# labRadioVision/federated

Hardware: AMD Instinct MI355X
Metric: device-resident GB/s, CFA reduce of K neighbour fp32 param buckets; 1/2/4/8 GPU (higher is better)
Workload: dtype f32

## Files before the change

### federated_amd/csrc/cfa_internal.h

```cpp
#pragma once
#include <hip/hip_runtime.h>

#include <cmath>
#include <cstdarg>
#include <cstdint>
#include <cstdio>
#include <cstdlib>
#include <cstring>
#include <string>
#include <type_traits>
#include <utility>

#include "cfa_engine.h"
#include "cfa_mix_shape.h"

typedef float f4 __attribute__((ext_vector_type(4)));
typedef unsigned u4v __attribute__((ext_vector_type(4)));

inline thread_local std::string g_last_error;

__attribute__((format(printf, 2, 3))) inline int fail(int code, const char* fmt, ...) {
  char buf[512];
  va_list ap;
  va_start(ap, fmt);
  vsnprintf(buf, sizeof(buf), fmt, ap);
  va_end(ap);
  g_last_error = buf;
  return code;
}

#define CFA_HIP_CHECK(expr)                                                              \
  do {                                                                                   \
    hipError_t e_ = (expr);                                                              \
    if (e_ != hipSuccess)                                                                \
      return fail(CFA_E_HIP, "%s failed: %s (%s:%d)", #expr, hipGetErrorString(e_),      \
                  __FILE__, __LINE__);                                                   \
  } while (0)

inline int check_launch(const char* what) {
  hipError_t e = hipGetLastError();
  if (e != hipSuccess) return fail(CFA_E_HIP, "%s launch failed: %s", what, hipGetErrorString(e));
  return CFA_OK;
}

namespace {

constexpr int kBlock = 256;

constexpr int kDefaultBlocks = 2;
constexpr int kAutoBlocks = -1;
static cfa_launch_t read_tune() {
  cfa_launch_t t{kAutoBlocks, 0, 1};
  if (const char* s = getenv("CFA_BLOCKS_PER_CU")) {
    const int v = atoi(s);
    t.blocks_per_cu = v >= 0 ? v : kAutoBlocks;
  }
  if (const char* s = getenv("CFA_VEC_PER_LANE")) t.vec_per_lane = norm_vec(atoi(s));
  if (const char* s = getenv("CFA_NONTEMPORAL")) t.nontemporal = atoi(s) ? 1 : 0;
  return t;
}
static const cfa_launch_t& tune() {
  static const cfa_launch_t t = read_tune();
  static const bool dynamic = getenv("CFA_TUNE_DYNAMIC") != nullptr;
  if (dynamic) {
    thread_local cfa_launch_t d;
    d = read_tune();
    return d;
  }
  return t;
}

}

inline int device_attr(int slot, hipDeviceAttribute_t attr, int fallback, bool keep_fallback) {
  static int cache[2][64] = {{0}};
  int dev = 0;
  if (hipGetDevice(&dev) != hipSuccess) return fallback;
  if (dev >= 0 && dev < 64) {
    const int c = __atomic_load_n(&cache[slot][dev], __ATOMIC_RELAXED);
    if (c > 0) return c;
  }
  int v = 0;
  if (hipDeviceGetAttribute(&v, attr, dev) != hipSuccess || v <= 0) {
    if (!keep_fallback) return fallback;
    v = fallback;
  }
  if (dev >= 0 && dev < 64) __atomic_store_n(&cache[slot][dev], v, __ATOMIC_RELAXED);
  return v;
}
inline int device_cus() { return device_attr(0, hipDeviceAttributeMultiprocessorCount, 256, false); }
inline int device_lds_max() { return device_attr(1, hipDeviceAttributeMaxSharedMemoryPerBlock, 65536, true); }

int grad_prepare_device();
int local_sgd_prepare_device();
int lenet_prepare_device();
int lenet_grad_prepare_device();
int advance_counter(unsigned long long* counter, hipStream_t st);

namespace {

static unsigned grid_for(long long tiles, const cfa_launch_t& t = tune()) {
  if (tiles <= 0) return 1;
  long long g = tiles;
  const int bpc = t.blocks_per_cu == kAutoBlocks ? kDefaultBlocks : t.blocks_per_cu;
  if (bpc > 0) {
    long long cap = (long long)device_cus() * bpc;
    if (g > cap) g = cap;
  }
  if (g > 0x7fffffffLL) g = 0x7fffffffLL;
  return (unsigned)g;
}

static unsigned grid_for_own(long long tiles, int own_blocks_per_cu) {
  cfa_launch_t t = tune();
  if (t.blocks_per_cu == kAutoBlocks) t.blocks_per_cu = own_blocks_per_cu;
  return grid_for(tiles, t);
}

static unsigned shared_grid_x(long long tiles, int wg_per_cu, long long gy) {
  long long gx = ((long long)device_cus() * wg_per_cu + gy - 1) / gy;
  if (gx > tiles) gx = tiles;
  if (gx < 1) gx = 1;
  return (unsigned)gx;
}

static int env_int(const char* name, int unset) {
  const char* s = getenv(name);
  return s ? atoi(s) : unset;
}

struct Fanin {
  const float* src[CFA_MAX_FANIN + 1];
  float c[CFA_MAX_FANIN + 1];
  float d[CFA_MAX_FANIN + 1];
  double rd[CFA_MAX_FANIN + 1];
};

constexpr int kFcSubnormal = 0x0090;
__device__ __forceinline__ f4 div4_rn(f4 a, double rb, bool& subnormal) {
  f4 q;
  q.x = (float)((double)a.x * rb);
  q.y = (float)((double)a.y * rb);
  q.z = (float)((double)a.z * rb);
  q.w = (float)((double)a.w * rb);
  subnormal = subnormal | __builtin_isfpclass(q.x, kFcSubnormal) | __builtin_isfpclass(q.y, kFcSubnormal) |
              __builtin_isfpclass(q.z, kFcSubnormal) | __builtin_isfpclass(q.w, kFcSubnormal);
  return q;
}
__device__ __forceinline__ f4 div4_ieee(f4 a, float b) {
  f4 q;
  q.x = a.x / b;
  q.y = a.y / b;
  q.z = a.z / b;
  q.w = a.w / b;
  return q;
}

inline void set_reciprocals(Fanin& f, int n) {
  for (int k = 0; k <= n; ++k) f.rd[k] = 1.0 / (double)f.d[k];
}

template <bool NT>
__device__ __forceinline__ f4 ld4(const float* p, long long i) {
  const f4* q = reinterpret_cast<const f4*>(p) + i;
  if constexpr (NT) return __builtin_nontemporal_load(q);
  else return *q;
}
template <bool NT>
__device__ __forceinline__ void st4(float* p, long long i, f4 v) {
  f4* q = reinterpret_cast<f4*>(p) + i;
  if constexpr (NT) __builtin_nontemporal_store(v, q);
  else *q = v;
}

template <typename T>
__device__ __forceinline__ T seq_step(T acc, T x, float a) {
  T t = x - acc;
  t = a * t;
  return acc + t;
}

template <bool IEEE, typename T>
__device__ __forceinline__ T div_step(T w, T x, float c, float d, double rd, bool& subnormal) {
  T t = x - w;
  t = c * t;
  if constexpr (!IEEE) t = div4_rn(t, rd, subnormal);
  else if constexpr (std::is_same_v<T, f4>) t = div4_ieee(t, d);
  else t = t / d;
  return w + t;
}

template <typename T>
__device__ __forceinline__ T lin_step(T w, T x, float c) {
  if constexpr (std::is_same_v<T, float>) {
    return fmaf(c, x, w);
  } else {
    w.x = fmaf(c, x.x, w.x);
    w.y = fmaf(c, x.y, w.y);
    w.z = fmaf(c, x.z, w.z);
    w.w = fmaf(c, x.w, w.w);
    return w;
  }
}

template <typename L>
__device__ __forceinline__ double tf1_first(L l, float x, double a) {
  const float d = x - (float)l;
  return (double)l + a * (double)d;
}
template <typename X>
__device__ __forceinline__ double tf1_step(double w, X x, double a) {
  return w + a * ((double)x - w);
}

__device__ __forceinline__ double ddiv_rn(double a, double b, double rb, bool fast) {
  const double aa = __builtin_fabs(a);
  if (fast && aa >= 0x1p-900 && aa <= 0x1p900) {
    const double q = a * rb;
    const double r = __builtin_fma(-q, b, a);
    return __builtin_fma(r, rb, q);
  }
  return a / b;
}
template <bool IEEE>
__device__ __forceinline__ double div_step_f64(double w, double x, double a, double d, double r, bool fast) {
  if constexpr (IEEE) return w + (a * (x - w)) / d;
  else return w + ddiv_rn(a * (x - w), d, r, fast);
}

template <typename T>
__device__ __forceinline__ T mewma_step(T& W, T g, const T& s_old, float rho, float one_minus_rho, T lr, bool init,
                                        bool filtered) {
  T s;
  if (init) {
    s = g;
  } else {
    const T t1 = rho * g;
    const T t2 = one_minus_rho * s_old;
    s = t1 + t2;
  }
  const T u = lr * (filtered ? s : g);
  W = W - u;
  return s;
}

__device__ __forceinline__ double scale(double c, double x, bool f32) {
  return f32 ? (double)((float)c * (float)x) : c * x;
}
__device__ __forceinline__ double mewma_step_f64(double& W, bool& w32, double g, const double& s_old, double rho,
                                                 double one_minus_rho, double lr, bool init, bool filtered,
                                                 bool s32, bool g32) {
  double s;
  if (init) {
    s = g;
  } else {
    const double t1 = scale(rho, g, g32);
    const double t2 = scale(one_minus_rho, s_old, s32);
    s = (g32 && s32) ? (double)((float)t1 + (float)t2) : t1 + t2;
  }
  if (s32) s = (double)(float)s;
  const bool u32 = filtered ? s32 : g32;
  const double t = scale(lr, filtered ? s : g, u32);
  if (w32 && u32) {
    W = (double)((float)W - (float)t);
  } else {
    W = W - t;
    w32 = false;
  }
  return s;
}

__device__ __forceinline__ float split_sum(const float* p, int n, long long stride) {
  float s = p[0];
  for (int sp = 1; sp < n; ++sp) s += p[(long long)sp * stride];
  return s;
}

template <int N, bool IEEE>
__device__ __forceinline__ f4 fold_div(const f4 (&v)[N + 1], const Fanin& f, bool& subnormal) {
  f4 w = v[0];
#pragma unroll
  for (int j = 1; j <= N; ++j) w = div_step<IEEE>(w, v[j], f.c[j], f.d[j], f.rd[j], subnormal);
  return w;
}

template <int N, int RULE>
__device__ __forceinline__ f4 fold(const f4 (&v)[N + 1], const Fanin& f) {
  if constexpr (RULE == CFA_RULE_SEQUENTIAL) {
    f4 w = v[0];
#pragma unroll
    for (int j = 1; j <= N; ++j) w = seq_step(w, v[j], f.c[j]);
    return w;
  } else if constexpr (RULE == CFA_RULE_SEQUENTIAL_DIV) {
    bool subnormal = false;
    f4 w = fold_div<N, false>(v, f, subnormal);
    if (__builtin_expect(subnormal, 0)) w = fold_div<N, true>(v, f, subnormal);
    return w;
  } else {
    f4 w = f.c[0] * v[0];
#pragma unroll
    for (int j = 1; j <= N; ++j) w = lin_step(w, v[j], f.c[j]);
    return w;
  }
}

template <int U>
struct TileWalk {
  static constexpr long long kTile = (long long)kBlock * U;
  long long nvec, full;
  __device__ explicit TileWalk(long long n) : nvec(n), full(n / kTile) {}
  struct Tiles {
    long long t, full;
    __device__ Tiles begin() const { return *this; }
    __device__ long long end() const { return full; }
    __device__ bool operator!=(long long e) const { return t < e; }
    __device__ void operator++() { t += gridDim.x; }
    __device__ long long operator*() const { return t * kTile + threadIdx.x; }
  };
  struct Vectors {
    long long i, nvec;
    __device__ Vectors begin() const { return *this; }
    __device__ long long end() const { return nvec; }
    __device__ bool operator!=(long long e) const { return i < e; }
    __device__ void operator++() { i += kBlock; }
    __device__ long long operator*() const { return i; }
  };
  __device__ Tiles full_tiles() const { return {(long long)blockIdx.x, full}; }
  __device__ bool owns_partial() const { return blockIdx.x == (unsigned)(full % gridDim.x); }
  __device__ Vectors partial_tile() const { return {full * kTile + threadIdx.x, nvec}; }
};

template <int LO, typename F, int... Is>
inline void dispatch_fanin_seq(int n, F&& fn, std::integer_sequence<int, Is...>) {
  ((n == LO + Is ? (void)fn(std::integral_constant<int, LO + Is>{}) : (void)0), ...);
}
template <int LO, typename F>
inline void dispatch_fanin(int n, F&& fn) {
  dispatch_fanin_seq<LO>(n, fn, std::make_integer_sequence<int, CFA_MAX_FANIN - LO + 1>{});
}

__device__ __forceinline__ double np_sign(double x) {
  return x > 0.0 ? 1.0 : (x < 0.0 ? -1.0 : x);
}
__device__ __forceinline__ float np_signf(float x) {
  return x > 0.0f ? 1.0f : (x < 0.0f ? -1.0f : x);
}
__device__ __forceinline__ float compress_one(float y, float ref, const CompressParams& cp,
                                              unsigned& kept) {
  const float thr = (float)cp.thr, rep = (float)cp.rep;
  if (cp.mode == CFA_COMPRESS_SPARSE || cp.mode == CFA_COMPRESS_SPARSE_HI) {
    if (fabsf(y) < thr) return np_signf(y) * rep;
  } else if (cp.mode == CFA_COMPRESS_SPARSE_DPCM || cp.mode == CFA_COMPRESS_SPARSE_DPCM_HI) {
    const float d = y - ref;
    if (fabsf(d) < thr) return ref + np_signf(d) * rep;
  }
  ++kept;
  return y;
}

__device__ __host__ constexpr int compress_kind(int mode) {
  return (mode == CFA_COMPRESS_SPARSE || mode == CFA_COMPRESS_SPARSE_HI) ? 1
         : (mode == CFA_COMPRESS_SPARSE_DPCM || mode == CFA_COMPRESS_SPARSE_DPCM_HI) ? 2 : 0;
}
template <int KIND>
__device__ __forceinline__ float compress_sel(float y, float ref, float thr, float rep, unsigned& kept) {
  if constexpr (KIND == 0) {
    ++kept;
    return y;
  } else {
    const float d = KIND == 2 ? y - ref : y;
    const bool hit = fabsf(d) < thr;
    const float r = KIND == 2 ? ref + np_signf(d) * rep : np_signf(y) * rep;
    kept += hit ? 0u : 1u;
    return hit ? r : y;
  }
}

__device__ __forceinline__ void block_add_count(unsigned kept, unsigned long long* dst) {
  __shared__ unsigned red[kBlock / 64];
  unsigned v = kept;
#pragma unroll
  for (int off = 32; off > 0; off >>= 1) v += __shfl_xor(v, off, 64);
  const int wave = threadIdx.x >> 6;
  if ((threadIdx.x & 63) == 0) red[wave] = v;
  __syncthreads();
  if (threadIdx.x == 0) {
    unsigned long long s = 0;
#pragma unroll
    for (int i = 0; i < kBlock / 64; ++i) s += red[i];
    if (s) atomicAdd(dst, s);
  }
}


constexpr long long kMaxChunkVec = 1LL << 27;
constexpr int kStoreSc1 = 16;
constexpr int kStoreNt = 2;

template <typename F>
inline void for_each_chunk(long long nvec, F&& fn) {
  for (long long done = 0; done < nvec; done += kMaxChunkVec)
    fn(done, (nvec - done) < kMaxChunkVec ? (nvec - done) : kMaxChunkVec);
}

__device__ __forceinline__ __amdgpu_buffer_rsrc_t out_rsrc(void* base, unsigned bytes) {
  return __builtin_amdgcn_make_buffer_rsrc(base, 0, bytes, 0x00020000);
}
template <int POLICY, typename V>
__device__ __forceinline__ void st16_buf(__amdgpu_buffer_rsrc_t r, long long idx, V v) {
  static_assert(sizeof(V) == 16, "16-byte vectors only");
  __builtin_amdgcn_raw_buffer_store_b128(__builtin_bit_cast(u4v, v), r, (int)(idx * 16), 0, POLICY);
}

struct Sc1Out {
  __amdgpu_buffer_rsrc_t r;
  void* base;
  bool buf;
};
__device__ __forceinline__ Sc1Out sc1_out(void* base, long long bytes) {
  Sc1Out o;
  o.base = base;
  o.buf = bytes <= 0x7FFFFFF0LL;
  o.r = out_rsrc(base, o.buf ? (unsigned)bytes : 0u);
  return o;
}
template <typename V>
__device__ __forceinline__ void st16_sc1(const Sc1Out& o, long long idx, V v) {
  if (o.buf)
    st16_buf<kStoreSc1>(o.r, idx, v);
  else
    __builtin_nontemporal_store(v, reinterpret_cast<V*>(o.base) + idx);
}

__device__ __forceinline__ double compress_one_d(double y, double ref, const CompressParams& cp,
                                                 unsigned& kept) {
  if (cp.mode == CFA_COMPRESS_SPARSE || cp.mode == CFA_COMPRESS_SPARSE_HI) {
    if (fabs(y) < cp.thr) return np_sign(y) * cp.rep;
  } else if (cp.mode == CFA_COMPRESS_SPARSE_DPCM || cp.mode == CFA_COMPRESS_SPARSE_DPCM_HI) {
    const double d = y - ref;
    if (fabs(d) < cp.thr) return ref + np_sign(d) * cp.rep;
  }
  ++kept;
  return y;
}

static inline uintptr_t addr(const void* p) { return reinterpret_cast<uintptr_t>(p); }

static int compress_params(int mode, CompressParams& cp) {
  cp.mode = mode;
  switch (mode) {
    case CFA_COMPRESS_NONE: cp.thr = 0.0; cp.rep = 0.0; break;
    case CFA_COMPRESS_SPARSE: cp.thr = 0.001; cp.rep = 0.0001; break;
    case CFA_COMPRESS_SPARSE_DPCM: cp.thr = 1.e-4; cp.rep = 1.e-4; break;
    case CFA_COMPRESS_SPARSE_DPCM_HI: cp.thr = 1.e-3; cp.rep = 1.e-3; break;
    case CFA_COMPRESS_SPARSE_HI: cp.thr = 0.01; cp.rep = 0.001; break;
    default: return fail(CFA_E_INVALID, "unknown compression mode %d", mode);
  }
  return CFA_OK;
}

static int validate_mix(const float* out, const float* local, const float* const* nbrs, int n,
                        size_t P) {
  if (n < 0) return fail(CFA_E_INVALID, "negative fan-in %d", n);
  if (P == 0) return CFA_OK;
  if (!out || !local) return fail(CFA_E_INVALID, "null out/local bucket");
  if (n > 0 && !nbrs) return fail(CFA_E_INVALID, "null neighbour table");
  for (int j = 0; j < n; ++j) {
    if (!nbrs[j]) return fail(CFA_E_INVALID, "null neighbour bucket %d", j);
    if (nbrs[j] == out) return fail(CFA_E_INVALID, "output aliases neighbour %d", j);
  }
  return CFA_OK;
}

static bool needs_ref(int mode) {
  return mode == CFA_COMPRESS_SPARSE_DPCM || mode == CFA_COMPRESS_SPARSE_DPCM_HI;
}

struct SchedArgs {
  const int32_t* sched;
  unsigned long long* round;
  unsigned S;
};

__device__ __forceinline__ int sched_slot(const SchedArgs& sc) {
  const unsigned long long r = *static_cast<const unsigned long long*>(sc.round);
  return sc.sched[r % sc.S];
}

__device__ __forceinline__ int first_flagged(const int32_t* flags, const int32_t* idx, int b, int e) {
  __shared__ int first;
  if (threadIdx.x == 0) first = e;
  __syncthreads();
  for (int k = b + (int)threadIdx.x; k < e; k += kBlock)
    if (flags[idx[k]]) {
      atomicMin(&first, k);
      break;
    }
  __syncthreads();
  return __builtin_amdgcn_readfirstlane(first);
}

static int sched_args(const int32_t* sched, int S, int T, unsigned long long* round, SchedArgs& sc) {
  if (S <= 0 || T <= 0) return fail(CFA_E_INVALID, "schedule of %d slots over %d tables", S, T);
  if (!sched || !round) return fail(CFA_E_INVALID, "null schedule or round counter");
  sc = SchedArgs{sched, round, (unsigned)S};
  return CFA_OK;
}
static int advance_round(const SchedArgs& sc, hipStream_t st) { return advance_counter(sc.round, st); }
}
```

### federated_amd/csrc/cfa_mix.hip

```cpp
#include <chrono>
#include <thread>

#include "cfa_internal.h"

extern "C" int cfa_version(void) { return CFA_VERSION; }

extern "C" int cfa_host_device_pointer(const void* host, void** dev) {
  if (!host || !dev) return fail(CFA_E_INVALID, "null pointer");
  *dev = nullptr;
  void* p = nullptr;
  hipError_t e = hipHostGetDevicePointer(&p, const_cast<void*>(host), 0);
  if (e != hipSuccess || !p)
    return fail(CFA_E_HIP, "hipHostGetDevicePointer: %s (not pinned host memory?)", hipGetErrorString(e));
  *dev = p;
  return CFA_OK;
}
extern "C" int cfa_device_prepare(int device) {
  int prev = 0;
  CFA_HIP_CHECK(hipGetDevice(&prev));
  if (device != prev) CFA_HIP_CHECK(hipSetDevice(device));
  (void)device_cus();
  int rc = grad_prepare_device();
  if (rc == CFA_OK) rc = local_sgd_prepare_device();
  if (rc == CFA_OK) rc = lenet_prepare_device();
  if (device != prev) CFA_HIP_CHECK(hipSetDevice(prev));
  return rc;
}
extern "C" int cfa_stream_synchronize(void* stream) {
  CFA_HIP_CHECK(hipStreamSynchronize((hipStream_t)stream));
  return CFA_OK;
}
extern "C" int cfa_memcpy_async(void* dst, const void* src, size_t bytes, void* stream) {
  if (bytes && (!dst || !src)) return fail(CFA_E_INVALID, "null copy pointer");
  if (bytes) CFA_HIP_CHECK(hipMemcpyAsync(dst, src, bytes, hipMemcpyDefault, (hipStream_t)stream));
  return CFA_OK;
}
extern "C" int cfa_counter_fetch(unsigned long long* counter, unsigned long long* host_dst, void* stream) {
  if (!counter || !host_dst) return fail(CFA_E_INVALID, "null counter or destination");
  hipStream_t st = (hipStream_t)stream;
  CFA_HIP_CHECK(hipMemcpyAsync(host_dst, counter, sizeof(*counter), hipMemcpyDefault, st));
  CFA_HIP_CHECK(hipMemsetAsync(counter, 0, sizeof(*counter), st));
  return CFA_OK;
}
namespace {
__global__ void stream_signal_kernel(unsigned* word, unsigned value) {
  __hip_atomic_store(word, value, __ATOMIC_RELEASE, __HIP_MEMORY_SCOPE_SYSTEM);
}
}
extern "C" int cfa_stream_signal(unsigned* word_dev, unsigned value, void* stream) {
  if (!word_dev) return fail(CFA_E_INVALID, "null signal word");
  stream_signal_kernel<<<1, 1, 0, (hipStream_t)stream>>>(word_dev, value);
  return check_launch("stream_signal");
}
extern "C" int cfa_host_wait_word(const unsigned* word_host, unsigned value, long long timeout_us) {
  if (!word_host) return fail(CFA_E_INVALID, "null wait word");
  if (timeout_us <= 0) return fail(CFA_E_INVALID, "timeout_us must be positive (got %lld)", timeout_us);
  auto reached = [&] { return static_cast<int>(__atomic_load_n(word_host, __ATOMIC_ACQUIRE) - value) >= 0; };
  if (reached()) return CFA_OK;
  const auto t0 = std::chrono::steady_clock::now();
  const auto spin = std::chrono::microseconds(20), limit = std::chrono::microseconds(timeout_us);
  for (unsigned i = 1;; ++i) {
    if (reached()) return CFA_OK;
    if ((i & 63) == 0) {
      const auto dt = std::chrono::steady_clock::now() - t0;
      if (dt > limit) break;
      if (dt > spin) std::this_thread::sleep_for(std::chrono::microseconds(20));
    } else {
      __builtin_ia32_pause();
    }
  }
  if (reached()) return CFA_OK;
  return fail(CFA_E_TIMEOUT, "wait word holds %u after %lld us, expected %u", __atomic_load_n(word_host, __ATOMIC_ACQUIRE),
              timeout_us, value);
}
extern "C" int cfa_host_register(void* host, size_t bytes) {
  if (!host || !bytes) return fail(CFA_E_INVALID, "null or empty host range");
  CFA_HIP_CHECK(hipHostRegister(host, bytes, hipHostRegisterMapped | hipHostRegisterPortable));
  return CFA_OK;
}
extern "C" int cfa_host_unregister(void* host) {
  if (!host) return fail(CFA_E_INVALID, "null host pointer");
  CFA_HIP_CHECK(hipHostUnregister(host));
  return CFA_OK;
}
extern "C" int cfa_wait_signal(const unsigned* word_host, unsigned value, void* stream, long long spin_us) {
  if (!word_host) return fail(CFA_E_INVALID, "null signal word");
  const auto t0 = std::chrono::steady_clock::now();
  for (unsigned i = 0;; ++i) {
    if (__atomic_load_n(word_host, __ATOMIC_ACQUIRE) == value) return CFA_OK;
    __builtin_ia32_pause();
    if ((i & 255) == 255 &&
        std::chrono::steady_clock::now() - t0 > std::chrono::microseconds(spin_us > 0 ? spin_us : 0))
      break;
  }
  CFA_HIP_CHECK(hipStreamSynchronize((hipStream_t)stream));
  if (__atomic_load_n(word_host, __ATOMIC_ACQUIRE) != value)
    return fail(CFA_E_INVALID, "signal word holds %u after the stream completed, expected %u",
                __atomic_load_n(word_host, __ATOMIC_ACQUIRE), value);
  return CFA_OK;
}
extern "C" const char* cfa_last_error(void) { return g_last_error.c_str(); }
extern "C" __attribute__((visibility("hidden"))) void cfa_internal_set_error(const char* msg) {
  g_last_error = msg ? msg : "";
}

namespace {

template <int N, int RULE, int U, int POL>
__global__ __launch_bounds__(kBlock) void mix_vec_kernel(float* out, Fanin f, long long nvec) {
  const __amdgpu_buffer_rsrc_t w = out_rsrc(out, (unsigned)(nvec * 16));
  const TileWalk<U> tw(nvec);
  for (const long long base : tw.full_tiles()) {
    f4 v[U][N + 1];
#pragma unroll
    for (int k = 0; k <= N; ++k)
#pragma unroll
      for (int u = 0; u < U; ++u) v[u][k] = ld4<(POL != 0)>(f.src[k], base + (long long)u * kBlock);
#pragma unroll
    for (int u = 0; u < U; ++u) {
      const f4 y = fold<N, RULE>(v[u], f);
      if constexpr (POL != 0)
        st16_buf<POL == 2 ? kStoreNt : kStoreSc1>(w, base + (long long)u * kBlock, y);
      else
        st4<false>(out, base + (long long)u * kBlock, y);
    }
  }
  if (tw.owns_partial()) {
    for (const long long i : tw.partial_tile()) {
      f4 v[N + 1];
#pragma unroll
      for (int k = 0; k <= N; ++k) v[k] = ld4<false>(f.src[k], i);
      st4<false>(out, i, fold<N, RULE>(v, f));
    }
  }
}

template <int N, int KIND>
__global__ __launch_bounds__(kBlock) void mix_vec_compress_kernel(float* out, Fanin f,
                                                                   long long nvec,
                                                                   CompressParams cp) {
  constexpr int U = (N + 1) * 4 <= 40 ? 4 : ((N + 1) * 2 <= 40 ? 2 : 1);
  constexpr long long kTile = (long long)kBlock * U;
  const Sc1Out o = sc1_out(out, nvec * 16);
  const float thr = (float)cp.thr, rep = (float)cp.rep;
  unsigned kept = 0;
  for (long long base = (long long)blockIdx.x * kTile + threadIdx.x; base < nvec;
       base += (long long)gridDim.x * kTile) {
    f4 v[U][N + 1];
#pragma unroll
    for (int k = 0; k <= N; ++k)
#pragma unroll
      for (int u = 0; u < U; ++u) {
        const long long i = base + (long long)u * kBlock;
        v[u][k] = i < nvec ? ld4<true>(f.src[k], i) : f4{0.f, 0.f, 0.f, 0.f};
      }
#pragma unroll
    for (int u = 0; u < U; ++u) {
      const long long i = base + (long long)u * kBlock;
      if (i >= nvec) continue;
      f4 w = fold<N, CFA_RULE_SEQUENTIAL>(v[u], f);
      const long long e0 = i * 4;
      if (e0 + 3 >= cp.cbegin && e0 < cp.cend) {
        const f4 r = v[u][0];
#pragma unroll
        for (int c = 0; c < 4; ++c) {
          const long long e = e0 + c;
          if (e >= cp.cbegin && e < cp.cend) w[c] = compress_sel<KIND>(w[c], r[c], thr, rep, kept);
        }
      }
      st16_sc1(o, i, w);
    }
  }
  block_add_count(kept, cp.kept);
}

struct ScalarFanin {
  const float* src[CFA_MAX_FANIN + 1];
  float c[CFA_MAX_FANIN + 1];
  float d[CFA_MAX_FANIN + 1];
  int n;
};
__global__ __launch_bounds__(kBlock) void mix_scalar_kernel(float* out, ScalarFanin f, long long P,
                                                            int rule, int compress,
                                                            CompressParams cp) {
  unsigned kept = 0;
  for (long long i = (long long)blockIdx.x * kBlock + threadIdx.x; i < P;
       i += (long long)gridDim.x * kBlock) {
    const float w0 = f.src[0][i];
    float w;
    if (rule == CFA_RULE_SEQUENTIAL) {
      w = w0;
      for (int j = 1; j <= f.n; ++j) w = seq_step(w, f.src[j][i], f.c[j]);
    } else if (rule == CFA_RULE_SEQUENTIAL_DIV) {
      w = w0;
      bool unused = false;
      for (int j = 1; j <= f.n; ++j) w = div_step<true>(w, f.src[j][i], f.c[j], f.d[j], 0.0, unused);
    } else {
      w = f.c[0] * w0;
      for (int j = 1; j <= f.n; ++j) w = lin_step(w, f.src[j][i], f.c[j]);
    }
    if (compress && i >= cp.cbegin && i < cp.cend) w = compress_one(w, w0, cp, kept);
    out[i] = w;
  }
  if (compress) block_add_count(kept, cp.kept);
}

template <int KIND>
__global__ __launch_bounds__(kBlock) void compress_kernel(float* y, const float* ref, long long P,
                                                          long long nvec, CompressParams cp) {
  unsigned kept = 0;
  const float thr = (float)cp.thr, rep = (float)cp.rep;
  constexpr int U = 4;
  f4* y4 = reinterpret_cast<f4*>(y);
  const f4* r4 = reinterpret_cast<const f4*>(ref);
  const TileWalk<U> tw(nvec);
  for (const long long base : tw.full_tiles()) {
    f4 v[U], r[U];
#pragma unroll
    for (int u = 0; u < U; ++u) {
      v[u] = y4[base + (long long)u * kBlock];
      if constexpr (KIND == 2) r[u] = r4[base + (long long)u * kBlock];
      else r[u] = f4{0.f, 0.f, 0.f, 0.f};
    }
#pragma unroll
    for (int u = 0; u < U; ++u) {
#pragma unroll
      for (int c = 0; c < 4; ++c) v[u][c] = compress_sel<KIND>(v[u][c], r[u][c], thr, rep, kept);
      y4[base + (long long)u * kBlock] = v[u];
    }
  }
  if (tw.owns_partial()) {
    for (const long long i : tw.partial_tile()) {
      f4 v = y4[i];
      const f4 r = (KIND == 2) ? r4[i] : f4{0.f, 0.f, 0.f, 0.f};
#pragma unroll
      for (int c = 0; c < 4; ++c) v[c] = compress_sel<KIND>(v[c], r[c], thr, rep, kept);
      y4[i] = v;
    }
  }
  const long long stride = (long long)gridDim.x * kBlock;
  for (long long i = 4 * nvec + (long long)blockIdx.x * kBlock + threadIdx.x; i < P; i += stride) {
    const float r = (KIND == 2) ? ref[i] : 0.0f;
    y[i] = compress_sel<KIND>(y[i], r, thr, rep, kept);
  }
  block_add_count(kept, cp.kept);
}

template <int RULE, int U, int POL>
static void launch_vec_u(int n, unsigned grid, hipStream_t st, float* out, const Fanin& f,
                         long long nvec) {
  dispatch_fanin<0>(n, [&](auto N) {
    mix_vec_kernel<decltype(N)::value, RULE, U, POL><<<grid, kBlock, 0, st>>>(out, f, nvec);
  });
}

template <int RULE>
static void launch_vec_chunk(int n, hipStream_t st, float* out, const Fanin& f, long long nvec,
                             const cfa_launch_t& t) {
  const bool own = t.blocks_per_cu == kAutoBlocks &&
                   (RULE == CFA_RULE_SEQUENTIAL || RULE == CFA_RULE_SEQUENTIAL_DIV);
  int own_bpc = 1, own_vec = 1;
  if (own) mix_auto_shape(n, nvec, own_bpc, own_vec);
  if (own && RULE == CFA_RULE_SEQUENTIAL_DIV && own_bpc == 1) own_vec = auto_vec(n);
  const int U = t.vec_per_lane > 0 ? norm_vec(t.vec_per_lane) : (own ? own_vec : auto_vec(n));
  const long long tiles = (nvec + (long long)kBlock * U - 1) / ((long long)kBlock * U);
  cfa_launch_t shape = t;
  if (own) shape.blocks_per_cu = own_bpc;
  const unsigned grid = grid_for(tiles, shape);
  const bool nt_store = own && shape.blocks_per_cu == 1 && nvec * 4 >= (8LL << 20) && t.nontemporal;
  if (U == 4) {
    if (t.nontemporal) launch_vec_u<RULE, 4, 1>(n, grid, st, out, f, nvec);
    else launch_vec_u<RULE, 4, 0>(n, grid, st, out, f, nvec);
  } else if (U == 2) {
    if constexpr (RULE == CFA_RULE_SEQUENTIAL)
      if (nt_store) return launch_vec_u<RULE, 2, 2>(n, grid, st, out, f, nvec);
    if (t.nontemporal) launch_vec_u<RULE, 2, 1>(n, grid, st, out, f, nvec);
    else launch_vec_u<RULE, 2, 0>(n, grid, st, out, f, nvec);
  } else {
    if constexpr (RULE == CFA_RULE_SEQUENTIAL)
      if (nt_store) return launch_vec_u<RULE, 1, 2>(n, grid, st, out, f, nvec);
    if (t.nontemporal) launch_vec_u<RULE, 1, 1>(n, grid, st, out, f, nvec);
    else launch_vec_u<RULE, 1, 0>(n, grid, st, out, f, nvec);
  }
}

template <int RULE>
static void launch_vec(int n, hipStream_t st, float* out, const Fanin& f, long long nvec,
                       const cfa_launch_t& t) {
  for_each_chunk(nvec, [&](long long done, long long m) {
    Fanin g = f;
    for (int k = 0; k <= n; ++k) g.src[k] = f.src[k] + done * 4;
    launch_vec_chunk<RULE>(n, st, out + done * 4, g, m, t);
  });
}

template <int KIND>
static void launch_vec_compress_k(int n, unsigned grid, hipStream_t st, float* out, const Fanin& f,
                                  long long nvec, const CompressParams& cp) {
  dispatch_fanin<0>(n, [&](auto N) {
    mix_vec_compress_kernel<decltype(N)::value, KIND><<<grid, kBlock, 0, st>>>(out, f, nvec, cp);
  });
}

static void launch_vec_compress(int n, hipStream_t st, float* out, const Fanin& f, long long nvec,
                                const CompressParams& cp) {
  const unsigned grid = grid_for((nvec + kBlock - 1) / kBlock);
  switch (compress_kind(cp.mode)) {
    case 1: launch_vec_compress_k<1>(n, grid, st, out, f, nvec, cp); break;
    case 2: launch_vec_compress_k<2>(n, grid, st, out, f, nvec, cp); break;
    default: launch_vec_compress_k<0>(n, grid, st, out, f, nvec, cp); break;
  }
}

static int mix_pass(float* out, const float* local, const float* const* nbrs, const float* c,
                    int n, size_t P, int rule, const CompressParams* cp, hipStream_t st,
                    const cfa_launch_t& lc = tune(), const float* div = nullptr) {
  const BucketSplit bs = bucket_split(
      n + 2, [&](int k) { return k == 0 ? addr(out) : (k == 1 ? addr(local) : addr(nbrs[k - 2])); }, P);
  const size_t head = bs.head, nvec = bs.nvec;

  CompressParams cpv{};
  if (cp) cpv = *cp;

  if (nvec > 0) {
    Fanin f{};
    f.src[0] = local + head;
    for (int j = 0; j < n; ++j) f.src[j + 1] = nbrs[j] + head;
    for (int k = 0; k <= n; ++k) f.c[k] = c[k];
    for (int k = 0; k <= n; ++k) f.d[k] = div ? div[k] : 1.0f;
    set_reciprocals(f, n);
    if (cp) {
      launch_vec_compress(n, st, out + head, f, (long long)nvec, shifted(cpv, (long long)head));
    } else if (rule == CFA_RULE_SEQUENTIAL) {
      launch_vec<CFA_RULE_SEQUENTIAL>(n, st, out + head, f, (long long)nvec, lc);
    } else if (rule == CFA_RULE_SEQUENTIAL_DIV) {
      launch_vec<CFA_RULE_SEQUENTIAL_DIV>(n, st, out + head, f, (long long)nvec, lc);
    } else {
      launch_vec<CFA_RULE_LINEAR>(n, st, out + head, f, (long long)nvec, lc);
    }
    if (int rc = check_launch("mix_vec")) return rc;
  }
  const size_t pieces[2][2] = {{0, head}, {bs.tail_begin, P}};
  for (auto& pc : pieces) {
    const size_t b = pc[0], e = pc[1];
    if (e <= b) continue;
    ScalarFanin sf{};
    sf.src[0] = local + b;
    for (int j = 0; j < n; ++j) {
      sf.src[j + 1] = nbrs[j] + b;
    }
    for (int k = 0; k <= n; ++k) sf.c[k] = c[k];
    for (int k = 0; k <= n; ++k) sf.d[k] = div ? div[k] : 1.0f;
    sf.n = n;
    const long long len = (long long)(e - b);
    mix_scalar_kernel<<<grid_for((len + kBlock - 1) / kBlock), kBlock, 0, st>>>(
        out + b, sf, len, rule, cp ? 1 : 0, shifted(cpv, (long long)b));
    if (int rc = check_launch("mix_scalar")) return rc;
  }
  return CFA_OK;
}

static int mix_seq_any(float* out, const float* local, const float* const* nbrs,
                       const float* alphas, int n, size_t P, const CompressParams* cp,
                       hipStream_t st, const cfa_launch_t& lc = tune()) {
  if (int rc = validate_mix(out, local, nbrs, n, P)) return rc;
  if (P == 0) return CFA_OK;
  const bool split_epilogue = cp && n > CFA_MAX_FANIN;
  if (split_epilogue && out == local && needs_ref(cp->mode))
    return fail(CFA_E_INVALID, "in-place DPCM compression needs fan-in <= %d", CFA_MAX_FANIN);
  const CompressParams* fused = (cp && !split_epilogue) ? cp : nullptr;
  const int rc = for_each_pass(n, [&](int done, int m, bool) {
    float c[CFA_MAX_FANIN + 1] = {1.0f};
    for (int j = 0; j < m; ++j) c[j + 1] = alphas[done + j];
    return mix_pass(out, done ? out : local, nbrs + done, c, m, P, CFA_RULE_SEQUENTIAL, fused, st, lc);
  }, true);
  if (rc) return rc;
  if (split_epilogue)
    return cfa_compress_epilogue_f32(out + cp->cbegin, local + cp->cbegin, cp->mode,
                                     (size_t)(cp->cend - cp->cbegin), cp->kept, st);
  return CFA_OK;
}

}

extern "C" int cfa_mix_seq_f32(float* out, const float* local, const float* const* nbrs,
                               const float* alphas, int n, size_t P, void* stream) {
  if (n > 0 && !alphas) return fail(CFA_E_INVALID, "null alphas");
  return mix_seq_any(out, local, nbrs, alphas, n, P, nullptr, (hipStream_t)stream);
}

extern "C" int cfa_mix_seq_ex_f32(float* out, const float* local, const float* const* nbrs,
                                  const float* alphas, int n, size_t P,
                                  const cfa_launch_t* launch, void* stream) {
  if (n > 0 && !alphas) return fail(CFA_E_INVALID, "null alphas");
  if (launch && launch->blocks_per_cu < 0) return fail(CFA_E_INVALID, "blocks_per_cu < 0");
  cfa_launch_t lc = launch ? *launch : tune();
  lc.vec_per_lane = norm_vec(lc.vec_per_lane);
  return mix_seq_any(out, local, nbrs, alphas, n, P, nullptr, (hipStream_t)stream, lc);
}

extern "C" int cfa_mix_seq_div_f32(float* out, const float* local, const float* const* nbrs,
                                   const float* alphas, const float* divisors, int n, size_t P,
                                   void* stream) {
  if (n > 0 && (!alphas || !divisors)) return fail(CFA_E_INVALID, "null alphas/divisors");
  if (int rc = validate_mix(out, local, nbrs, n, P)) return rc;
  if (P == 0) return CFA_OK;
  hipStream_t st = (hipStream_t)stream;
  return for_each_pass(n, [&](int done, int m, bool) {
    float c[CFA_MAX_FANIN + 1] = {1.0f}, d[CFA_MAX_FANIN + 1] = {1.0f};
    for (int j = 0; j < m; ++j) {
      c[j + 1] = alphas[done + j];
      d[j + 1] = divisors[done + j];
    }
    return mix_pass(out, done ? out : local, nbrs + done, c, m, P, CFA_RULE_SEQUENTIAL_DIV, nullptr, st, tune(), d);
  }, true);
}

extern "C" int cfa_mix_f32(float* out, const float* local, const float* const* nbrs,
                           const float* coeff, int n, size_t P, void* stream) {
  if (!coeff) return fail(CFA_E_INVALID, "null coefficients");
  if (int rc = validate_mix(out, local, nbrs, n, P)) return rc;
  if (P == 0) return CFA_OK;
  hipStream_t st = (hipStream_t)stream;
  return for_each_pass(n, [&](int done, int m, bool) {
    float c[CFA_MAX_FANIN + 1] = {done == 0 ? coeff[0] : 1.0f};
    for (int j = 0; j < m; ++j) c[j + 1] = coeff[done + j + 1];
    return mix_pass(out, done ? out : local, nbrs + done, c, m, P, CFA_RULE_LINEAR, nullptr, st);
  }, true);
}

extern "C" int cfa_mix_seq_compress_f32(float* out, const float* local, const float* const* nbrs,
                                        const float* alphas, int n, size_t P, int mode,
                                        size_t cbegin, size_t cend,
                                        unsigned long long* kept_count, void* stream) {
  if (n > 0 && !alphas) return fail(CFA_E_INVALID, "null alphas");
  if (!kept_count) return fail(CFA_E_INVALID, "null kept_count");
  if (cbegin > cend || cend > P) return fail(CFA_E_INVALID, "bad compression range");
  CompressParams cp{};
  if (int rc = compress_params(mode, cp)) return rc;
  cp.cbegin = (long long)cbegin;
  cp.cend = (long long)cend;
  cp.kept = kept_count;
  hipStream_t st = (hipStream_t)stream;
  if (n == 0) {
    if (out != local && P > 0)
      CFA_HIP_CHECK(hipMemcpyAsync(out, local, P * sizeof(float), hipMemcpyDefault, st));
    return cfa_compress_epilogue_f32(out + cbegin, local + cbegin, mode, cend - cbegin,
                                     kept_count, stream);
  }
  return mix_seq_any(out, local, nbrs, alphas, n, P, &cp, st);
}

extern "C" int cfa_compress_epilogue_f32(float* y, const float* ref, int mode, size_t P,
                                         unsigned long long* kept_count, void* stream) {
  if (!kept_count) return fail(CFA_E_INVALID, "null kept_count");
  CompressParams cp{};
  if (int rc = compress_params(mode, cp)) return rc;
  if ((mode == CFA_COMPRESS_SPARSE_DPCM || mode == CFA_COMPRESS_SPARSE_DPCM_HI) && !ref && P)
    return fail(CFA_E_INVALID, "DPCM compression needs a reference bucket");
  if (P == 0) return CFA_OK;
  if (!y) return fail(CFA_E_INVALID, "null bucket");
  cp.cbegin = 0;
  cp.cend = (long long)P;
  cp.kept = kept_count;
  hipStream_t st = (hipStream_t)stream;
  const bool vec = (addr(y) & 15) == 0 && (!ref || (addr(ref) & 15) == 0);
  const long long nvec = vec ? (long long)P / 4 : 0;
  const unsigned grid = grid_for(((vec ? nvec : (long long)P) + kBlock - 1) / kBlock);
  switch (compress_kind(mode)) {
    case 1: compress_kernel<1><<<grid, kBlock, 0, st>>>(y, ref, (long long)P, nvec, cp); break;
    case 2: compress_kernel<2><<<grid, kBlock, 0, st>>>(y, ref, (long long)P, nvec, cp); break;
    default: compress_kernel<0><<<grid, kBlock, 0, st>>>(y, ref, (long long)P, nvec, cp); break;
  }
  return check_launch("compress");
}
```

### federated_amd/csrc/cfa_ring.hip

```cpp
#include <type_traits>

#include "cfa_internal.h"
#include "cfa_slide_shape.h"

namespace {

constexpr int kWinMaxDev = 8;
struct WindowArgs {
  const float* rows[kWinMaxDev + 8];
  float* out[kWinMaxDev];
  float a[kWinMaxDev];
  int nb;
};

template <int HL, int HR, typename Row>
__device__ __forceinline__ f4 ring_fold(Row row, float a) {
  f4 acc = row(HL);
#pragma unroll
  for (int j = 0; j < HL; ++j) acc = seq_step(acc, row(j), a);
#pragma unroll
  for (int j = 0; j < HR; ++j) acc = seq_step(acc, row(HL + 1 + j), a);
  return acc;
}

template <int HL, int HR, int U, bool SC1>
__device__ __forceinline__ void window_body(const WindowArgs& w, long long nvec) {
  constexpr int R = kWinMaxDev + HL + HR;
  constexpr long long kTile = (long long)kBlock * U;
  const int nr = w.nb + HL + HR;
  for (long long t = blockIdx.x; t * kTile < nvec; t += gridDim.x) {
    const long long base = t * kTile + threadIdx.x;
    f4 r[U][R];
#pragma unroll
    for (int k = 0; k < R; ++k)
      if (k < nr)
#pragma unroll
        for (int u = 0; u < U; ++u) {
          const long long i = base + (long long)u * kBlock;
          if (i < nvec) r[u][k] = ld4<true>(w.rows[k], i);
        }
#pragma unroll
    for (int b = 0; b < kWinMaxDev; ++b)
      if (b < w.nb) {
        const __amdgpu_buffer_rsrc_t o = out_rsrc(w.out[b], (unsigned)(nvec * 16));
#pragma unroll
        for (int u = 0; u < U; ++u) {
          const long long i = base + (long long)u * kBlock;
          if (i < nvec) {
            const f4 y = ring_fold<HL, HR>([&](int j) { return r[u][b + j]; }, w.a[b]);
            if constexpr (SC1)
              st16_buf<kStoreSc1>(o, i, y);
            else
              st4<true>(w.out[b], i, y);
          }
        }
      }
  }
}

template <int HL, int HR, int U, bool SC1>
__global__ __launch_bounds__(kBlock) void window_vec_kernel(WindowArgs w, long long nvec) {
  window_body<HL, HR, U, SC1>(w, nvec);
}

struct RingArgs {
  const float* in;
  float* out;
  const float* alphas;
  long long pitch;
  long long off;
  int D;
};

template <int HL, int HR, int U, bool SC1>
__global__ __launch_bounds__(kBlock) void ring_round_kernel(RingArgs ra, long long nvec) {
  const int p = blockIdx.y;
  WindowArgs w;
  w.nb = min(kWinMaxDev, ra.D - p * kWinMaxDev);
#pragma unroll
  for (int k = 0; k < kWinMaxDev + HL + HR; ++k) {
    const int g = ((p * kWinMaxDev - HL + k) % ra.D + ra.D) % ra.D;
    w.rows[k] = ra.in + (long long)g * ra.pitch + ra.off;
  }
#pragma unroll
  for (int b = 0; b < kWinMaxDev; ++b) {
    const int d = min(p * kWinMaxDev + b, ra.D - 1);
    w.out[b] = ra.out + (long long)d * ra.pitch + ra.off;
    w.a[b] = ra.alphas[d];
  }
  window_body<HL, HR, U, SC1>(w, nvec);
}

struct SlideArgs {
  const float* in;
  float* out;
  const float* alphas;
  long long in_pitch, out_pitch;
  long long off;
  int rows, first, count, seg;
};

template <int HL, int HR, int PF, int U, bool SC1>
__global__ __launch_bounds__(kBlock) void ring_slide_kernel(SlideArgs sa, long long nvec) {
  constexpr int W = HL + HR + 1;
  constexpr int RS = W + PF;
  constexpr long long kTile = (long long)kBlock * U;
  const int n0 = (int)blockIdx.y * sa.seg;
  const int len = min(sa.seg, sa.count - n0);
  const int total = len + HL + HR;
  const int d0 = sa.first + n0;
  int g0 = (d0 - HL) % sa.rows;
  if (g0 < 0) g0 += sa.rows;
  const int o0 = d0 >= sa.rows ? d0 - sa.rows : d0;
  const float* const in = sa.in + sa.off;
  float* const out = sa.out + sa.off;
  const float* const in_end = in + (long long)sa.rows * sa.in_pitch;
  float* const out_end = out + (long long)sa.rows * sa.out_pitch;
  for (long long t = blockIdx.x; t * kTile < nvec; t += gridDim.x) {
    const long long i = t * kTile + threadIdx.x;
    if (i >= nvec) continue;
    bool ok[U];
    unsigned voff[U];
#pragma unroll
    for (int v = 0; v < U; ++v) {
      ok[v] = i + (long long)v * kBlock < nvec;
      voff[v] = (unsigned)((ok[v] ? i + (long long)v * kBlock : i) * 16);
    }
    const float* rp = in + (long long)g0 * sa.in_pitch;
    float* op = out + (long long)o0 * sa.out_pitch;
    f4 r[RS][U];
    auto load_row = [&](f4(&slot)[U]) {
#pragma unroll
      for (int v = 0; v < U; ++v)
        slot[v] = __builtin_nontemporal_load(reinterpret_cast<const f4*>(reinterpret_cast<const char*>(rp) + voff[v]));
      rp += sa.in_pitch;
      if (rp == in_end) rp = in;
    };
#pragma unroll
    for (int q = 0; q < RS - 1; ++q)
      if (q < total) load_row(r[q]);
    for (int n = 0; n < len; n += RS) {
#pragma unroll
      for (int u = 0; u < RS; ++u) {
        const int m = n + u;
        if (m < len) {
          if (m + RS - 1 < total) load_row(r[(u + RS - 1) % RS]);
          const float a = sa.alphas[n0 + m];
          f4 acc[U];
#pragma unroll
          for (int v = 0; v < U; ++v) acc[v] = ring_fold<HL, HR>([&](int j) { return r[(u + j) % RS][v]; }, a);
#pragma unroll
          for (int v = 0; v < U; ++v)
            if (ok[v]) {
              if constexpr (SC1)
                st16_buf<kStoreSc1>(out_rsrc(op, (unsigned)(nvec * 16)), i + (long long)v * kBlock, acc[v]);
              else
                __builtin_nontemporal_store(acc[v], reinterpret_cast<f4*>(reinterpret_cast<char*>(op) + voff[v]));
            }
          op += sa.out_pitch;
          if (op == out_end) op = out;
        }
      }
    }
  }
}

__global__ __launch_bounds__(kBlock) void window_scalar_kernel(WindowArgs w, int hl, int hr,
                                                               long long begin, long long P) {
  for (long long i = begin + (long long)blockIdx.x * kBlock + threadIdx.x; i < P;
       i += (long long)gridDim.x * kBlock) {
    for (int b = 0; b < w.nb; ++b) {
      float acc = w.rows[b + hl][i];
      for (int j = 0; j < hl; ++j) acc = seq_step(acc, w.rows[b + j][i], w.a[b]);
      for (int j = 0; j < hr; ++j) acc = seq_step(acc, w.rows[b + hl + 1 + j][i], w.a[b]);
      w.out[b][i] = acc;
    }
  }
}

}

namespace {
struct WindowTune {
  int vec, sc1, blocks_per_cu;
};
static WindowTune window_tune() {
  WindowTune t{1, 0, 6};
  t.vec = env_int("CFA_WINDOW_VEC", t.vec) == 1 ? 1 : 2;
  t.sc1 = env_int("CFA_WINDOW_SC1", t.sc1) ? 1 : 0;
  t.blocks_per_cu = env_int("CFA_WINDOW_BLOCKS_PER_CU", t.blocks_per_cu);
  if (t.blocks_per_cu <= 0) t.blocks_per_cu = 2;
  return t;
}
static long long window_tiles(long long m, const WindowTune& t) {
  return (m + (long long)kBlock * t.vec - 1) / ((long long)kBlock * t.vec);
}
template <typename F>
void for_vec_sc1(const WindowTune& t, F&& fn) {
  using One = std::integral_constant<int, 1>;
  using Two = std::integral_constant<int, 2>;
  if (t.vec == 1) {
    if (t.sc1) fn(One{}, std::true_type{});
    else fn(One{}, std::false_type{});
  } else {
    if (t.sc1) fn(Two{}, std::true_type{});
    else fn(Two{}, std::false_type{});
  }
}
template <int HL, int HR>
void launch_window(const WindowArgs& w, long long nvec, hipStream_t st) {
  const WindowTune t = window_tune();
  const cfa_launch_t lc{t.blocks_per_cu, t.vec, 1};
  for_each_chunk(nvec, [&](long long done, long long m) {
    WindowArgs c = w;
    for (int k = 0; k < w.nb + HL + HR; ++k) c.rows[k] = w.rows[k] + done * 4;
    for (int b = 0; b < w.nb; ++b) c.out[b] = w.out[b] + done * 4;
    const unsigned grid = grid_for(window_tiles(m, t), lc);
    for_vec_sc1(t, [&](auto u, auto sc1) {
      window_vec_kernel<HL, HR, decltype(u)::value, decltype(sc1)::value><<<grid, kBlock, 0, st>>>(c, m);
    });
  });
}
template <int HL, int HR>
void launch_ring_round(const RingArgs& ra, long long nvec, hipStream_t st) {
  const WindowTune t = window_tune();
  const cfa_launch_t lc{t.blocks_per_cu, t.vec, 1};
  const unsigned passes = (unsigned)((ra.D + kWinMaxDev - 1) / kWinMaxDev);
  for_each_chunk(nvec, [&](long long done, long long m) {
    RingArgs c = ra;
    c.off = ra.off + done * 4;
    const long long tiles = window_tiles(m, t);
    long long gx = (grid_for(tiles, lc) + passes - 1) / passes;
    if (gx < 1) gx = 1;
    if (gx > tiles) gx = tiles;
    const dim3 grid((unsigned)gx, passes);
    for_vec_sc1(t, [&](auto u, auto sc1) {
      ring_round_kernel<HL, HR, decltype(u)::value, decltype(sc1)::value><<<grid, kBlock, 0, st>>>(c, m);
    });
  });
}

static_assert(kSlideBlock == kBlock, "cfa_slide_shape.h counts tiles of kBlock lanes");
static SlideTune slide_tune() {
  const SlideTune d = kSlideDefault;
  SlideTune t{env_int("CFA_SLIDE_SEGMENTS", d.segments), env_int("CFA_SLIDE_WG_PER_CU", d.wg_per_cu),
              env_int("CFA_SLIDE_PF", d.pf), env_int("CFA_SLIDE_SC1", d.sc1) ? 1 : 0, env_int("CFA_SLIDE_U", 0)};
  if (t.segments <= 0) t.segments = d.segments;
  if (t.wg_per_cu <= 0) t.wg_per_cu = d.wg_per_cu;
  if (t.pf < 1 || t.pf > 2) t.pf = d.pf;
  if (t.u != 1 && t.u != 2 && t.u != 4) t.u = 0;
  return t;
}
template <int HL, int HR, int PF, int U>
void launch_slide_shape(const SlideArgs& c, long long m, dim3 grid, bool sc1, hipStream_t st) {
  if (sc1) ring_slide_kernel<HL, HR, PF, U, true><<<grid, kBlock, 0, st>>>(c, m);
  else ring_slide_kernel<HL, HR, PF, U, false><<<grid, kBlock, 0, st>>>(c, m);
}
template <int HL, int HR, int U>
void launch_slide_u(const SlideArgs& c, long long m, dim3 grid, const SlideTune& t, hipStream_t st) {
  switch (t.pf) {
    case 1: launch_slide_shape<HL, HR, 1, U>(c, m, grid, t.sc1, st); break;
    default: launch_slide_shape<HL, HR, 2, U>(c, m, grid, t.sc1, st); break;
  }
}
template <int HL, int HR>
void launch_ring_slide(const SlideArgs& sa, long long nvec, hipStream_t st) {
  const SlideTune t = slide_tune();
  int segments = t.segments < sa.count ? t.segments : sa.count;
  if (segments > 65535) segments = 65535;
  SlideArgs c = sa;
  c.seg = (sa.count + segments - 1) / segments;
  const unsigned gy = (unsigned)((sa.count + c.seg - 1) / c.seg);
  for_each_chunk(nvec, [&](long long done, long long m) {
    c.off = done * 4;
    const int u = t.u ? t.u : slide_pick_u(m, kSlideDefault.u, device_cus(), t.wg_per_cu);
    const dim3 grid(shared_grid_x(slide_tiles(m, u), t.wg_per_cu, gy), gy);
    switch (u) {
      case 4: launch_slide_u<HL, HR, 4>(c, m, grid, t, st); break;
      case 2: launch_slide_u<HL, HR, 2>(c, m, grid, t, st); break;
      default: launch_slide_u<HL, HR, 1>(c, m, grid, t, st); break;
    }
  });
}

#define CFA_HLHR_ROW(F, L) {&F<L, 0>, &F<L, 1>, &F<L, 2>, &F<L, 3>, &F<L, 4>}
#define CFA_HLHR_TABLE(F) \
  {CFA_HLHR_ROW(F, 0), CFA_HLHR_ROW(F, 1), CFA_HLHR_ROW(F, 2), CFA_HLHR_ROW(F, 3), CFA_HLHR_ROW(F, 4)}
void (*const kWindowLaunch[5][5])(const WindowArgs&, long long, hipStream_t) = CFA_HLHR_TABLE(launch_window);
void (*const kRingLaunch[5][5])(const RingArgs&, long long, hipStream_t) = CFA_HLHR_TABLE(launch_ring_round);
void (*const kSlideLaunch[5][5])(const SlideArgs&, long long, hipStream_t) = CFA_HLHR_TABLE(launch_ring_slide);
#undef CFA_HLHR_TABLE
#undef CFA_HLHR_ROW
}

extern "C" int cfa_mix_window_f32(float* const* out, const float* const* rows, const float* alphas,
                                  int nb, int hl, int hr, size_t P, void* stream) {
  if (nb < 1 || nb > kWinMaxDev) return fail(CFA_E_INVALID, "nb %d outside 1..%d", nb, kWinMaxDev);
  if (hl < 0 || hr < 0 || hl > 4 || hr > 4) return fail(CFA_E_INVALID, "window %d/%d outside 0..4", hl, hr);
  if (!out || !rows || !alphas) return fail(CFA_E_INVALID, "null table");
  if (P == 0) return CFA_OK;
  WindowArgs w{};
  w.nb = nb;
  const int nr = nb + hl + hr;
  bool aligned = true;
  for (int k = 0; k < nr; ++k) {
    if (!rows[k]) return fail(CFA_E_INVALID, "null row %d", k);
    w.rows[k] = rows[k];
    aligned = aligned && (addr(rows[k]) & 15) == 0;
  }
  for (int b = 0; b < nb; ++b) {
    if (!out[b]) return fail(CFA_E_INVALID, "null output %d", b);
    for (int k = 0; k < nr; ++k)
      if (out[b] == rows[k]) return fail(CFA_E_INVALID, "output %d aliases row %d", b, k);
    w.out[b] = out[b];
    aligned = aligned && (addr(out[b]) & 15) == 0;
    w.a[b] = alphas[b];
  }
  hipStream_t st = (hipStream_t)stream;
  const long long nvec = aligned ? (long long)(P / 4) : 0;
  if (nvec > 0) {
    kWindowLaunch[hl][hr](w, nvec, st);
    if (int rc = check_launch("window_vec")) return rc;
  }
  const long long begin = nvec * 4;
  if (begin < (long long)P) {
    const long long len = (long long)P - begin;
    window_scalar_kernel<<<grid_for((len + kBlock - 1) / kBlock), kBlock, 0, st>>>(w, hl, hr, begin, (long long)P);
    if (int rc = check_launch("window_scalar")) return rc;
  }
  return CFA_OK;
}

extern "C" int cfa_mix_ring_round_f32(float* out, const float* in, size_t pitch, const float* alphas, int D,
                                      int hl, int hr, size_t P, void* stream) {
  if (D < 1) return fail(CFA_E_INVALID, "device count %d", D);
  if (hl < 0 || hr < 0 || hl > 4 || hr > 4) return fail(CFA_E_INVALID, "window %d/%d outside 0..4", hl, hr);
  if (hl + hr >= D) return fail(CFA_E_INVALID, "window %d/%d wider than %d devices", hl, hr, D);
  if (!out || !in || !alphas) return fail(CFA_E_INVALID, "null buffer");
  if (pitch < P) return fail(CFA_E_INVALID, "pitch %zu below P %zu", pitch, P);
  if (P == 0) return CFA_OK;
  if ((addr(out) & 15) || (addr(in) & 15) || (pitch % 4) || (P % 4))
    return fail(CFA_E_UNSUPPORTED, "ring round needs 16-byte aligned rows (pitch and P multiples of 4)");
  const long long outb = (long long)addr(out), inb = (long long)addr(in), span = (long long)D * (long long)pitch * 4;
  if (outb < inb + span && inb < outb + span) return fail(CFA_E_INVALID, "out overlaps in");
  if ((long long)(D + kWinMaxDev - 1) / kWinMaxDev > 65535) return fail(CFA_E_INVALID, "D=%d exceeds grid.y", D);
  RingArgs ra{in, out, alphas, (long long)pitch, 0, D};
  kRingLaunch[hl][hr](ra, (long long)(P / 4), (hipStream_t)stream);
  return check_launch("ring_round");
}

extern "C" int cfa_mix_ring_slide_f32(float* out, size_t out_pitch, const float* in, size_t in_pitch,
                                      const float* alphas, int rows, int first, int count, int hl, int hr,
                                      size_t P, void* stream) {
  if (!out || !in || !alphas) return fail(CFA_E_INVALID, "null buffer");
  if (rows < 1 || count < 1) return fail(CFA_E_INVALID, "rows %d / count %d below 1", rows, count);
  if (first < 0 || first >= rows || count > rows || (count != rows && first > rows - count))
    return fail(CFA_E_INVALID, "devices %d..%d outside a ring of %d rows", first, first + count - 1, rows);
  if (hl < 0 || hr < 0 || hl > 4 || hr > 4) return fail(CFA_E_INVALID, "window %d/%d outside 0..4", hl, hr);
  if (hl + hr >= rows) return fail(CFA_E_INVALID, "window %d/%d wider than %d rows", hl, hr, rows);
  if (in_pitch < P || out_pitch < P)
    return fail(CFA_E_INVALID, "pitch %zu/%zu below P %zu", out_pitch, in_pitch, P);
  if (P == 0) return CFA_OK;
  const unsigned long long outb = addr(out), inb = addr(in);
  const unsigned long long out_span = ((unsigned long long)(rows - 1) * out_pitch + P) * 4;
  const unsigned long long in_span = ((unsigned long long)(rows - 1) * in_pitch + P) * 4;
  if (outb < inb + in_span && inb < outb + out_span) return fail(CFA_E_INVALID, "out overlaps in");
  if ((outb & 15) || (inb & 15) || (out_pitch % 4) || (in_pitch % 4) || (P % 4))
    return fail(CFA_E_UNSUPPORTED, "ring slide needs 16-byte aligned rows (pitches and P multiples of 4)");
  SlideArgs sa{in, out, alphas, (long long)in_pitch, (long long)out_pitch, 0, rows, first, count, count};
  kSlideLaunch[hl][hr](sa, (long long)(P / 4), (hipStream_t)stream);
  return check_launch("ring_slide");
}
```

### federated_amd/csrc/cfa_slide_shape.h

```cpp
#pragma once

constexpr int kSlideBlock = 256;

struct SlideTune {
  int segments, wg_per_cu, pf, sc1, u;
};
constexpr SlideTune kSlideDefault{1, 4, 2, 0, 4};

inline long long slide_tiles(long long nvec, int u) {
  const long long tile = (long long)kSlideBlock * u;
  return (nvec + tile - 1) / tile;
}

inline int slide_pick_u(long long nvec, int want, int cus, int wg_per_cu) {
  int u = want >= 4 ? 4 : (want >= 2 ? 2 : 1);
  while (u > 1 && slide_tiles(nvec, u) < (long long)cus * wg_per_cu) u >>= 1;
  return u;
}
```

Baseline: 25670.

## Reuse first ring rows from registers/LDS at wraparound seam in slide kernel

For a full-ring slide with one segment, the kernel stashes the first K=HL+HR input rows in registers and LDS after loading them, then serves the wraparound rows from there instead of re-reading them from global memory. This removes K redundant row reads per tile, cutting HBM traffic when the ring is small. In exchange it uses dynamic LDS (with an attribute raise above 64KB), sets launch bounds that constrain occupancy and adds a separate kernel instantiation with a device prepare hook.

New measurement: 26130, median of 6. 1.8% higher.

```diff
diff --git a/federated_amd/csrc/cfa_internal.h b/federated_amd/csrc/cfa_internal.h
--- a/federated_amd/csrc/cfa_internal.h
+++ b/federated_amd/csrc/cfa_internal.h
@@ -95,6 +95,7 @@
 int local_sgd_prepare_device();
 int lenet_prepare_device();
 int lenet_grad_prepare_device();
+int ring_prepare_device();
 int advance_counter(unsigned long long* counter, hipStream_t st);
 
 namespace {
diff --git a/federated_amd/csrc/cfa_mix.hip b/federated_amd/csrc/cfa_mix.hip
--- a/federated_amd/csrc/cfa_mix.hip
+++ b/federated_amd/csrc/cfa_mix.hip
@@ -23,6 +23,7 @@
   int rc = grad_prepare_device();
   if (rc == CFA_OK) rc = local_sgd_prepare_device();
   if (rc == CFA_OK) rc = lenet_prepare_device();
+  if (rc == CFA_OK) rc = ring_prepare_device();
   if (device != prev) CFA_HIP_CHECK(hipSetDevice(prev));
   return rc;
 }
diff --git a/federated_amd/csrc/cfa_ring.hip b/federated_amd/csrc/cfa_ring.hip
--- a/federated_amd/csrc/cfa_ring.hip
+++ b/federated_amd/csrc/cfa_ring.hip
@@ -100,10 +100,18 @@
   int rows, first, count, seg;
 };
 
-template <int HL, int HR, int PF, int U, bool SC1>
-__global__ __launch_bounds__(kBlock) void ring_slide_kernel(SlideArgs sa, long long nvec) {
+__device__ __forceinline__ f4* slide_seam_lds() {
+  extern __shared__ __attribute__((aligned(16))) f4 seam_lds[];
+  return seam_lds;
+}
+
+template <int HL, int HR, int PF, int U, bool SC1, bool SEAM = false>
+__global__ __launch_bounds__(kBlock, SEAM ? slide_seam_waves(U) : 1) void ring_slide_kernel(SlideArgs sa,
+                                                                                            long long nvec) {
   constexpr int W = HL + HR + 1;
   constexpr int RS = W + PF;
+  constexpr int K = HL + HR;
+  constexpr int KV = SEAM ? K - slide_seam_lds_rows(K) : 0;
   constexpr long long kTile = (long long)kBlock * U;
   const int n0 = (int)blockIdx.y * sa.seg;
   const int len = min(sa.seg, sa.count - n0);
@@ -139,12 +147,42 @@
 #pragma unroll
     for (int q = 0; q < RS - 1; ++q)
       if (q < total) load_row(r[q]);
+    [[maybe_unused]] f4 keep[KV > 0 ? KV : 1][U];
+    if constexpr (SEAM) {
+#pragma unroll
+      for (int q = 0; q < K; ++q)
+#pragma unroll
+        for (int v = 0; v < U; ++v) {
+          if (q < KV) keep[q][v] = r[q][v];
+          else slide_seam_lds()[((q - KV) * U + v) * kBlock + threadIdx.x] = r[q][v];
+        }
+    }
     for (int n = 0; n < len; n += RS) {
 #pragma unroll
       for (int u = 0; u < RS; ++u) {
         const int m = n + u;
         if (m < len) {
-          if (m + RS - 1 < total) load_row(r[(u + RS - 1) % RS]);
+          if constexpr (SEAM) {
+            if (m + RS - 1 >= len) {
+              const int j = m + RS - 1 - len;
+              f4(&slot)[U] = r[(u + RS - 1) % RS];
+              if (j >= K) {
+              } else if (j >= KV) {
+#pragma unroll
+                for (int v = 0; v < U; ++v) slot[v] = slide_seam_lds()[((j - KV) * U + v) * kBlock + threadIdx.x];
+              } else {
+#pragma unroll
+                for (int k = 0; k < KV; ++k)
+                  if (j == k)
+#pragma unroll
+                    for (int v = 0; v < U; ++v) slot[v] = keep[k][v];
+              }
+            } else {
+              load_row(r[(u + RS - 1) % RS]);
+            }
+          } else {
+            if (m + RS - 1 < total) load_row(r[(u + RS - 1) % RS]);
+          }
           const float a = sa.alphas[n0 + m];
           f4 acc[U];
 #pragma unroll
@@ -263,9 +301,38 @@
     default: launch_slide_shape<HL, HR, 2, U>(c, m, grid, t.sc1, st); break;
   }
 }
+template <int HL, int HR, int U>
+bool slide_seam_lds_ready() {
+  constexpr int bytes = slide_seam_lds_bytes(HL + HR, U);
+  if constexpr (bytes > 65536) {
+    static unsigned long long raised = 0;
+    int dev = 0;
+    if (hipGetDevice(&dev) != hipSuccess || dev < 0 || dev >= 64) return false;
+    if (__atomic_load_n(&raised, __ATOMIC_RELAXED) >> dev & 1) return true;
+    if (bytes > device_lds_max() ||
+        hipFuncSetAttribute(reinterpret_cast<const void*>(&ring_slide_kernel<HL, HR, 1, U, false, true>),
+                            hipFuncAttributeMaxDynamicSharedMemorySize, bytes) != hipSuccess) {
+      (void)hipGetLastError();
+      return false;
+    }
+    __atomic_fetch_or(&raised, 1ULL << dev, __ATOMIC_RELAXED);
+  }
+  return true;
+}
+template <int HL, int HR, int U>
+bool launch_slide_seam(const SlideArgs& c, long long m, dim3 grid, hipStream_t st) {
+  if constexpr (HL + HR >= 1) {
+    if (!slide_seam_lds_ready<HL, HR, U>()) return false;
+    ring_slide_kernel<HL, HR, 1, U, false, true><<<grid, kBlock, slide_seam_lds_bytes(HL + HR, U), st>>>(c, m);
+    return true;
+  } else {
+    return false;
+  }
+}
 template <int HL, int HR>
 void launch_ring_slide(const SlideArgs& sa, long long nvec, hipStream_t st) {
   const SlideTune t = slide_tune();
+  const bool seam_wanted = env_int("CFA_SLIDE_SEAM", kSlideSeamDefault) != 0 && !t.sc1;
   int segments = t.segments < sa.count ? t.segments : sa.count;
   if (segments > 65535) segments = 65535;
   SlideArgs c = sa;
@@ -275,6 +342,9 @@
     c.off = done * 4;
     const int u = t.u ? t.u : slide_pick_u(m, kSlideDefault.u, device_cus(), t.wg_per_cu);
     const dim3 grid(shared_grid_x(slide_tiles(m, u), t.wg_per_cu, gy), gy);
+    if (seam_wanted && slide_takes_seam(sa.rows, sa.count, (int)gy, HL, HR, u) &&
+        (u == 4 ? launch_slide_seam<HL, HR, 4>(c, m, grid, st) : launch_slide_seam<HL, HR, 2>(c, m, grid, st)))
+      return;
     switch (u) {
       case 4: launch_slide_u<HL, HR, 4>(c, m, grid, t, st); break;
       case 2: launch_slide_u<HL, HR, 2>(c, m, grid, t, st); break;
@@ -289,8 +359,19 @@
 void (*const kWindowLaunch[5][5])(const WindowArgs&, long long, hipStream_t) = CFA_HLHR_TABLE(launch_window);
 void (*const kRingLaunch[5][5])(const RingArgs&, long long, hipStream_t) = CFA_HLHR_TABLE(launch_ring_round);
 void (*const kSlideLaunch[5][5])(const SlideArgs&, long long, hipStream_t) = CFA_HLHR_TABLE(launch_ring_slide);
+template <int HL, int HR>
+void slide_seam_prepare() {
+  if constexpr (HL + HR >= 1) (void)(slide_seam_lds_ready<HL, HR, 4>() && slide_seam_lds_ready<HL, HR, 2>());
+}
+void (*const kSlideSeamPrepare[5][5])() = CFA_HLHR_TABLE(slide_seam_prepare);
 #undef CFA_HLHR_TABLE
 #undef CFA_HLHR_ROW
+}
+
+int ring_prepare_device() {
+  for (int hl = 0; hl <= 4; ++hl)
+    for (int hr = 0; hr <= 4; ++hr) kSlideSeamPrepare[hl][hr]();
+  return CFA_OK;
 }
 
 extern "C" int cfa_mix_window_f32(float* const* out, const float* const* rows, const float* alphas,
diff --git a/federated_amd/csrc/cfa_slide_shape.h b/federated_amd/csrc/cfa_slide_shape.h
--- a/federated_amd/csrc/cfa_slide_shape.h
+++ b/federated_amd/csrc/cfa_slide_shape.h
@@ -17,3 +17,13 @@
   while (u > 1 && slide_tiles(nvec, u) < (long long)cus * wg_per_cu) u >>= 1;
   return u;
 }
+
+constexpr int kSlideSeamDefault = 1;
+constexpr int kSlideSeamLdsRows = 5;
+constexpr int slide_seam_lds_rows(int k) { return k < kSlideSeamLdsRows ? k : kSlideSeamLdsRows; }
+constexpr int slide_seam_lds_bytes(int k, int u) { return slide_seam_lds_rows(k) * u * kSlideBlock * 16; }
+constexpr int slide_seam_waves(int u) { return u >= 4 ? 2 : 4;  }
+
+inline bool slide_takes_seam(int rows, int count, int segments, int hl, int hr, int u) {
+  return count == rows && segments == 1 && hl + hr >= 1 && (u == 2 || u == 4);
+}
```
